# yangzichuang/TextSummarization-On-Flink

Measured on AMD Instinct MI355X. Metric: train_tokens_per_sec, higher is better.
Workload: dtype bf16; 1 GPU; model=pointer-generator+coverage hidden=256 emb=128 enc=400 dec=100 vocab=50000, global_batch=256, per_gpu_batch=256, seq_len=400->100, parallelism=dp1, backend=none, grad_allreduce=none, graph=True, persistent_lstm=True, proj_attn=True, skip_pad_steps=True, decoder_row_groups=2

## Files before the change

### csrc/bindings.cpp

```cpp
#include <torch/library.h>
#include <ATen/ATen.h>
#include <c10/hip/HIPStream.h>
#include <algorithm>
#include <optional>

#include "launchers.h"

using at::Tensor;
using OT = std::optional<Tensor>;

namespace {

hipStream_t stream() { return c10::hip::getCurrentHIPStream().stream(); }

void chk(const Tensor& t, at::ScalarType dt, const char* name) {
  TORCH_CHECK(t.is_cuda(), name, " must be a GPU tensor");
  TORCH_CHECK(t.scalar_type() == dt, name, " has dtype ", t.scalar_type(), ", expected ", dt);
  TORCH_CHECK(t.is_contiguous(), name, " must be contiguous");
}
template <typename T>
T* P(const Tensor& t) { return reinterpret_cast<T*>(t.data_ptr()); }
template <typename T>
T* PO(const OT& t) { return t.has_value() && t->defined() ? reinterpret_cast<T*>(t->data_ptr()) : nullptr; }
void numel_eq(const Tensor& t, int64_t n, const char* name) {
// ... 444 lines not shown
}


void dec_cell_fwd(const Tensor& XG, const OT& ctxp, const Tensor& hprev, const Tensor& cprev, const Tensor& WcT,
                  const Tensor& c_out, const Tensor& cb_out, const Tensor& hb_out, const Tensor& act, int64_t B,
                  int64_t H, int64_t A, const OT& dlen, int64_t step) {
  chk(XG, F32, "XG"); chk(hprev, BF, "hprev"); chk(cprev, F32, "cprev"); chk(WcT, BF, "WcT"); chk(c_out, F32, "c_out");
  chk(cb_out, BF, "cb_out"); chk(hb_out, BF, "hb_out"); chk(act, F32, "act");
  TORCH_CHECK(H % 32 == 0 && A % 32 == 0, "dims must be multiples of 32");
  numel_eq(XG, B * 4 * H, "XG"); chko(ctxp, BF, B * A, "ctxp"); numel_eq(hprev, B * H, "hprev");
  numel_eq(cprev, B * H, "cprev"); numel_eq(WcT, 4 * H * (A + H), "WcT"); numel_eq(c_out, B * H, "c_out");
  numel_eq(cb_out, B * H, "cb_out"); numel_eq(hb_out, B * H, "hb_out"); numel_eq(act, B * 4 * H, "act");
  chko(dlen, I32, B, "dlen");
  launch_dec_cell_fwd(P<float>(XG), PO<bf16>(ctxp), P<bf16>(hprev), P<float>(cprev), P<bf16>(WcT), P<float>(c_out),
                      P<bf16>(cb_out), P<bf16>(hb_out), P<float>(act), B, H, A, PO<int>(dlen), (int)step, stream());
}

void dec_sproj(const Tensor& cb, const Tensor& hb, const Tensor& WsT, const Tensor& bs, const Tensor& s_out, int64_t B,
               int64_t H, int64_t A, const OT& dlen, int64_t step) {
  chk(cb, BF, "cb"); chk(hb, BF, "hb"); chk(WsT, BF, "WsT"); chk(bs, F32, "bs"); chk(s_out, F32, "s_out");
  TORCH_CHECK(H % 32 == 0 && A % 16 == 0, "bad dims");
  numel_eq(cb, B * H, "cb"); numel_eq(hb, B * H, "hb"); numel_eq(WsT, A * 2 * H, "WsT"); numel_eq(bs, A, "bs");
  numel_eq(s_out, B * A, "s_out"); chko(dlen, I32, B, "dlen");
  launch_dec_sproj(P<bf16>(cb), P<bf16>(hb), P<bf16>(WsT), P<float>(bs), P<float>(s_out), B, H, A, PO<int>(dlen),
                   (int)step, stream());
}

void dec_bwd_cell(const Tensor& ds, const Tensor& Ws, const OT& dC_dir, const OT& dH_dir, const Tensor& dh_rec,
                  const Tensor& dc_carry, const Tensor& act, const Tensor& c_now, const Tensor& c_prev,
                  const Tensor& dz, int64_t B, int64_t H, int64_t A, const OT& dlen, int64_t step) {
  chk(ds, F32, "ds"); chk(Ws, BF, "Ws"); chk(dh_rec, F32, "dh_rec"); chk(dc_carry, F32, "dc_carry");
  chk(act, F32, "act"); chk(c_now, F32, "c_now"); chk(c_prev, F32, "c_prev"); chk(dz, BF, "dz");
  TORCH_CHECK(H % 16 == 0 && A % 32 == 0, "bad dims");
  numel_eq(ds, B * A, "ds"); numel_eq(Ws, 2 * H * A, "Ws"); chko(dC_dir, F32, B * H, "dC_dir");
  chko(dH_dir, F32, B * H, "dH_dir"); numel_eq(dh_rec, B * H, "dh_rec"); numel_eq(dc_carry, B * H, "dc_carry");
  numel_eq(act, B * 4 * H, "act"); numel_eq(c_now, B * H, "c_now"); numel_eq(c_prev, B * H, "c_prev");
  numel_eq(dz, B * 4 * H, "dz"); chko(dlen, I32, B, "dlen");
  launch_dec_bwd_cell(P<float>(ds), P<bf16>(Ws), PO<float>(dC_dir), PO<float>(dH_dir), P<float>(dh_rec),
                      P<float>(dc_carry), P<float>(act), P<float>(c_now), P<float>(c_prev), P<bf16>(dz), B, H, A,
                      PO<int>(dlen), (int)step, stream());
}

void dec_bwd_dz(const Tensor& dz, const Tensor& Wbig, const OT& dX_dir, const OT& dCTX_dir_prev, const Tensor& dx_out,
                const OT& dctx_prev_out, const Tensor& dh_rec, int64_t B, int64_t E, int64_t H, int64_t A,
                const OT& dlen, int64_t step) {
  chk(dz, BF, "dz"); chk(Wbig, BF, "Wbig"); chk(dx_out, F32, "dx_out"); chk(dh_rec, F32, "dh_rec");
  TORCH_CHECK(E % 16 == 0 && H % 32 == 0 && A % 16 == 0, "bad dims");
  numel_eq(dz, B * 4 * H, "dz"); numel_eq(Wbig, (E + H + A) * 4 * H, "Wbig");
  chko(dX_dir, F32, B * E, "dX_dir"); chko(dCTX_dir_prev, F32, B * A, "dCTX_dir_prev");
  numel_eq(dx_out, B * E, "dx_out"); chko(dctx_prev_out, F32, B * A, "dctx_prev_out");
  numel_eq(dh_rec, B * H, "dh_rec"); chko(dlen, I32, B, "dlen");
  launch_dec_bwd_dz(P<bf16>(dz), P<bf16>(Wbig), PO<float>(dX_dir), PO<float>(dCTX_dir_prev), P<float>(dx_out),
                    PO<float>(dctx_prev_out), P<float>(dh_rec), B, E, H, A, PO<int>(dlen), (int)step, stream());
}

void ptr_loss(const Tensor& logits, const OT& bias, const Tensor& target, const Tensor& rowg, const OT& pgen,
              const OT& attn, const Tensor& ext, const Tensor& lens, const Tensor& loss_row, const OT& dlogits,
              const OT& dpre, const OT& dA, int64_t N, int64_t B, int64_t T, int64_t V) {
  const bool lbf = logits.scalar_type() == at::kBFloat16;
  chk(logits, lbf ? BF : F32, "logits"); chk(target, I32, "target"); chk(rowg, F32, "rowg"); chk(ext, I32, "ext");
  chk(lens, I32, "lens"); chk(loss_row, F32, "loss_row");
  TORCH_CHECK(lbf != bias.has_value(), "bf16 logits carry their bias (pass None); fp32 logits need the bias");
  chko(bias, F32, V, "bias");
  numel_eq(logits, N * V, "logits"); numel_eq(target, N, "target"); numel_eq(rowg, N, "rowg");
  numel_eq(ext, B * T, "ext"); numel_eq(lens, B, "lens"); numel_eq(loss_row, N, "loss_row");
  TORCH_CHECK(N % B == 0, "N must be D*B");
  chko(pgen, F32, N, "pgen"); chko(attn, F32, N * T, "attn"); chko(dlogits, BF, N * V, "dlogits");
  chko(dpre, F32, N, "dpre"); chko(dA, F32, N * T, "dA");
  TORCH_CHECK(!PO<float>(pgen) || (PO<float>(attn) && (!PO<bf16>(dlogits) || (PO<float>(dpre) && PO<float>(dA)))),
              "pointer mode needs attn, and dpre/dA when computing grads");
  if (lbf) {
    TORCH_CHECK(V <= ptr_loss_bf16_max_vocab(), "bf16 ptr_loss: V <= 65536");
    launch_ptr_loss_bf16(P<bf16>(logits), P<int>(target), P<float>(rowg), PO<float>(pgen), PO<float>(attn),
                         P<int>(ext), P<int>(lens), P<float>(loss_row), PO<bf16>(dlogits), PO<float>(dpre),
                         PO<float>(dA), N, B, T, V, stream());
    return;
  }
  launch_ptr_loss(P<float>(logits), P<float>(*bias), P<int>(target), P<float>(rowg), PO<float>(pgen), PO<float>(attn),
                  P<int>(ext), P<int>(lens), P<float>(loss_row), PO<bf16>(dlogits), PO<float>(dpre), PO<float>(dA), N,
                  B, T, V, stream());
}

int64_t wgrad_tt_ws(int64_t M, int64_t N, int64_t K) {
  if (wgrad_tt_ok((int)M, (int)N, (int)K))
    return wgrad_tt_direct((int)M, (int)N, (int)K, false, false) ? 1
                                                                 : (int64_t)wgrad_tt_splits((int)M, (int)N, (int)K) * M * N;
  if (wgrad_tt_ok((int)N, (int)M, (int)K)) return (int64_t)wgrad_tt_splits((int)N, (int)M, (int)K) * M * N;
  return 0;
}
bool wgrad_tt(const Tensor& a, const Tensor& b, const Tensor& out, const Tensor& ws, bool acc) {
  TORCH_CHECK(a.dim() == 2 && b.dim() == 2 && out.dim() == 2, "wgrad_tt: 2-D views");
  TORCH_CHECK(a.is_cuda() && b.is_cuda() && out.is_cuda() && ws.is_cuda(), "wgrad_tt: GPU tensors");
  TORCH_CHECK(a.scalar_type() == BF && b.scalar_type() == BF && out.scalar_type() == F32 && ws.scalar_type() == F32,
              "wgrad_tt: bf16, bf16 -> fp32");
  TORCH_CHECK(a.stride(1) == 1 && b.stride(1) == 1 && out.stride(1) == 1 && ws.is_contiguous(), "wgrad_tt: unit column stride");
  const int64_t K = a.size(0), M = a.size(1), N = b.size(1), nv = out.size(1);
  TORCH_CHECK(b.size(0) == K && out.size(0) == M && nv <= N, "wgrad_tt: shapes");
  if (!(a.stride(0) % 8 == 0 && b.stride(0) % 8 == 0 && (uintptr_t)a.data_ptr() % 16 == 0 &&
        (uintptr_t)b.data_ptr() % 16 == 0))
    return false;
  const bool plain = wgrad_tt_ok((int)M, (int)N, (int)K), swapped = !plain && wgrad_tt_ok((int)N, (int)M, (int)K);
  if (!plain && !(swapped && nv == N)) return false;
  if (nv != N && (nv % 4 != 0)) return false;
  const bool direct = plain && wgrad_tt_direct((int)M, (int)N, (int)K, false, acc);
  const int64_t need = direct ? 0 : (int64_t)wgrad_tt_splits((int)(plain ? M : N), (int)(plain ? N : M), (int)K) * M * N;
  if (ws.numel() < need) {
// ... 699 lines not shown
  auto part = at::empty({S, Kt}, gw.options());
  auto cpart = at::empty({(int64_t)colsum_det_chunks((int)S, (int)Kt), Kt}, gw.options());
  launch_pgen_bwd(P<float>(ctx), P<float>(c), P<bf16>(h), P<float>(x), P<float>(dpre), P<float>(gw), P<float>(part),
                  P<float>(cpart), N, A, H, E, stream());
}

void pgen_dirs(const Tensor& dpre, const Tensor& w, const Tensor& dctx, const Tensor& dc, const Tensor& dh,
               const Tensor& dx, const OT& gb, int64_t N, int64_t A, int64_t H, int64_t E) {
  chk(dpre, F32, "dpre"); chk(w, F32, "w"); chk(dctx, F32, "dctx"); chk(dc, F32, "dc"); chk(dh, F32, "dh");
  chk(dx, F32, "dx"); chko(gb, F32, 1, "gb");
  numel_eq(dpre, N, "dpre"); numel_eq(w, A + 2 * H + E, "w"); numel_eq(dctx, N * A, "dctx"); numel_eq(dc, N * H, "dc");
  numel_eq(dh, N * H, "dh"); numel_eq(dx, N * E, "dx");
  launch_pgen_dirs(P<float>(dpre), P<float>(w), P<float>(dctx), P<float>(dc), P<float>(dh), P<float>(dx), PO<float>(gb),
                   (int)N, (int)A, (int)H, (int)E, stream());
}

}

TORCH_LIBRARY(tsamd, m) {
  m.def("lstm_enc_fwd_step", &lstm_enc_fwd_step);
  m.def("lstm_enc_bwd_step", &lstm_enc_bwd_step);
  m.def("lstm_persistent_grid", &lstm_persistent_grid_op);
  m.def("lstm_persistent_capacity", &lstm_persistent_capacity_op);
  m.def("lstm_persistent_launches", &lstm_persistent_launches_op);
  m.def("rs_fwd", &rs_fwd);
  m.def("vocab_topk_pg", &vocab_topk_pg);
  m.def("rs_bwd", &rs_bwd);
  m.def("lstm_persistent_xbuf", &lstm_persistent_xbuf_op);
  m.def("lstm_fwd_persistent", &lstm_fwd_persistent);
  m.def("lstm_fwd_persistent_fx", &lstm_fwd_persistent_fx);
  m.def("lstm_persistent_fx_ok", &lstm_persistent_fx_ok_op);
  m.def("lstm_bwd_persistent", &lstm_bwd_persistent);
  m.def("attn_score", &attn_score);
  m.def("attn_softmax_ctx", &attn_softmax_ctx);
  m.def("attn_bwd_step", &attn_bwd_step);
  m.def("attn_row_ok", &attn_row_ok);
  m.def("attn_fwd_row", &attn_fwd_row);
  m.def("attn_bwd_row", &attn_bwd_row);
  m.def("attn_rowp_ok", &attn_rowp_ok);
  m.def("attn_fwd_rowp", &attn_fwd_rowp);
  m.def("dec_persistent_ok", &dec_persistent_ok_op);
  m.def("dec_persistent_grid", &dec_persistent_grid_op);
  m.def("dec_persistent_capacity", &dec_persistent_capacity_op);
  m.def("dec_persistent_xbuf", &dec_persistent_xbuf_op);
  m.def("dec_persistent_stamps", &dec_persistent_stamps_op);
  m.def("dec_fwd_persistent", &dec_fwd_persistent);
  m.def("attn_bwd_rowp", &attn_bwd_rowp);
  m.def("attn_bwd_feat", &attn_bwd_feat);
  m.def("attn_chunks", &attn_chunks);
  m.def("dec_cell_fwd", &dec_cell_fwd);
  m.def("dec_sproj", &dec_sproj);
  m.def("dec_bwd_cell", &dec_bwd_cell);
  m.def("dec_bwd_dz", &dec_bwd_dz);
  m.def("ptr_loss", &ptr_loss);
  m.def("wgrad_tn", &wgrad_tn);
  m.def("wgrad_tt", &wgrad_tt);
  m.def("ctx_bmm_ok", &ctx_bmm_ok_op);
  m.def("ctx_fwd", &ctx_fwd);
  m.def("ctx_da", &ctx_da);
  m.def("ctx_de", &ctx_de);
  m.def("wgrad_tt_ws", &wgrad_tt_ws);
  m.def("pgen_dirs", &pgen_dirs);
  m.def("pack_cast", &pack_cast);
  m.def("pack_max_jobs", &pack_max_jobs_op);
  m.def("pack_job_cols", &pack_job_cols_op);
  m.def("debug_enabled", &debug_enabled);
  m.def("debug_status", &debug_status);
  m.def("debug_clear", &debug_clear);
  m.def("gemm_bt_ok", &gemm_bt_ok);
  m.def("gemm_bt", &gemm_bt);
  m.def("gemm_bt_splitk_ws", &gemm_bt_splitk_ws);
  m.def("gemm_bt_splitk", &gemm_bt_splitk);
  m.def("gemm_bt_merge", &gemm_bt_merge);
  m.def("cu_hold_max_lds", &cu_hold_max_lds_op);
  m.def("cu_hold", &cu_hold);
  m.def("tanh_eval", &tanh_eval);
  m.def("tanh_tput", &tanh_tput);
  m.def("vocab_train_tiles", &vocab_train_tiles_op);
  m.def("vocab_train_fwd", &vocab_train_fwd);
  m.def("vocab_train_bwd", &vocab_train_bwd);
  m.def("emb_grad", &emb_grad);
  m.def("emb_grad_sorted", &emb_grad_sorted);
  m.def("emb_grad_det", &emb_grad_det);
  m.def("emb_grad_det_chunks", &emb_grad_det_chunks_op);
  m.def("to_step_frame", &to_step_frame);
  m.def("from_step_frame", &from_step_frame);
  m.def("transpose_bta", &transpose_bta);
  m.def("tr01", &tr01);
  m.def("linear2_pair", &linear2_pair);
  m.def("cast_colsum", &cast_colsum);
  m.def("colsum", &colsum);
  m.def("step_frame_hop", &step_frame_hop);
  m.def("ptr_rowfin", &ptr_rowfin);
  m.def("clip_adagrad", &clip_adagrad);
  m.def("opt_parts", &opt_parts);
  m.def("final_topk", &final_topk);
  m.def("final_topk_wide", &final_topk_wide);
  m.def("topk_parts", &topk_parts);
  m.def("beam_step", &beam_step);
  m.def("beam_step_wide", &beam_step_wide);
  m.def("beam_step_ng", &beam_step_ng);
  m.def("beam_step_pen", &beam_step_pen);
  m.def("cov_penalty", &cov_penalty);
  m.def("beam_gather", &beam_gather);
  m.def("linear2", &linear2);
  m.def("pgen", &pgen);
// ... 15 lines not shown
```

### csrc/kernels/launchers.h

```cpp
#pragma once
#include <hip/hip_runtime.h>
typedef __bf16 bf16;

void launch_lstm_enc_fwd_step(const float* gx, const float* bias, const bf16* Wt, bf16* hs, float* cs, float* acts, bf16* out,
                              const int* lens, int s, int T, int B, int H, hipStream_t st);
void launch_lstm_enc_bwd_step(bf16* dz, const bf16* Wn, const float* dout, const float* dh_fin, float* dc_carry,
                              const float* acts, const float* cs, const int* lens, int s, int T, int B, int H,
                              hipStream_t st);

void launch_attn_score(const bf16* F, const float* s, const float* v, const float* wc, const float* cov,
                       const int* lens, float* e, int B, int T, int A, int rep, hipStream_t st);
void launch_attn_softmax_ctx(const float* e, const bf16* E, const int* lens, const float* cov, float* a_out,
                             float* cov_out, float* covloss, float* ctx, bf16* ctx_bf, int B, int T, int A, int rep,
                             hipStream_t st);
int attn_nchunk(int T);
void launch_attn_bwd_step(const bf16* E, const bf16* F, const float* s, const float* v, const float* wc,
                          const float* cov, const float* a, const float* dctx, const float* ctx, const float* Ga,
                          const float* dcov_next, const float* gcl, const int* lens, float* de_out, float* ds,
                          float* dcov_out, int B, int T, int A, hipStream_t st);
void launch_attn_bwd_feat(const bf16* F, const float* S_all, const float* v, const float* wc, const float* cov_all,
                          const float* de_all, const int* lens, bf16* dF, float* dv, float* dwc, int D, int B, int T,
                          int A, int nslot, hipStream_t st, const int* dlen = nullptr);

bool attn_row_supported(int A, int T);
void launch_attn_fwd_row_probe(const bf16* F, const bf16* E, const float* s, const float* v, const float* wc,
                               const float* cov, const int* lens, float* a_out, float* ctx, int B, int T, int rep,
                               int probe, hipStream_t st);
void launch_attn_fwd_row(const bf16* F, const bf16* E, const float* s, const float* v, const float* wc,
                         const float* cov, const int* lens, float* a_out, float* cov_out, float* covloss, float* ctx,
                         bf16* ctx_bf, int B, int T, int A, int rep, hipStream_t st, const int* cg = nullptr,
                         const float* asrc = nullptr, float* cov_keep = nullptr);
void launch_attn_bwd_row(const bf16* E, const bf16* F, const float* s, const float* v, const float* wc,
                         const float* cov, const float* a, const float* dctx, const float* ctx, const float* Ga,
                         const float* dcov_next, const float* gcl, const int* lens, float* de_out, float* ds,
                         float* dcov_out, int B, int T, int A, hipStream_t st);

bool attn_rowp_supported(int A, int T, int EG);
void launch_attn_fwd_rowp(const bf16* F, const bf16* G, const float* s, const float* v, const float* wc,
                          const float* cov, const int* lens, float* a_out, float* cov_out, float* covloss, float* gx,
                          bf16* gx_bf, int B, int T, int A, const int* dlen, int step, hipStream_t st,
                          bf16* a_bf = nullptr);
void launch_attn_bwd_rowp(const bf16* G, const bf16* F, const float* s, const float* v, const float* wc,
                          const float* cov, const float* a, const float* dx, const float* gv, const float* Ga,
                          const float* dcov_next, const float* gcl, const int* lens, float* de_out, float* ds,
                          float* dcov_out, int B, int T, int A, const int* dlen, int step, hipStream_t st);

void launch_dec_cell_fwd(const float* XG, const bf16* ctxp, const bf16* hprev, const float* cprev, const bf16* WcT,
                         float* c_out, bf16* cb_out, bf16* hb_out, float* act, int B, int H, int A, const int* dlen,
                         int step, hipStream_t st);
void launch_dec_cell_fwd_beam(const int* gidx, const int* latest, const float* XGtab, const bf16* ctxp,
                              const bf16* hprev, const float* cprev, const bf16* WcT, float* c_out, bf16* cb_out,
                              bf16* hb_out, int* step, int B, int H, int A, int V, int unk, hipStream_t st);
void launch_beam_sproj_xmerge(const bf16* cb, const bf16* hb, const bf16* WsT, const float* bs, float* s_out,
                              const bf16* ctx_src, const bf16* WicT, const float* Xtab, const int* gidx,
                              const int* latest, float* x_out, int B, int H, int A, int E, int V, int unk,
                              hipStream_t st);
void launch_dec_sproj(const bf16* cb, const bf16* hb, const bf16* WsT, const float* bs, float* s_out, int B, int H,
                      int A, const int* dlen, int step, hipStream_t st);
bool dec_persistent_shape_ok(int H, int E, int A, int B, int T);
int dec_persistent_grid(int B);
int dec_persistent_capacity();
size_t dec_persistent_xbuf_elems(int B);
int dec_persistent_stamps_into(unsigned* buf);
void launch_dec_fwd_persistent(const float* XG, const bf16* KcT, const bf16* WsT, const float* bs, float* Cst, bf16* Cb,
                               bf16* Hb, float* ACT, float* S, const bf16* F, const bf16* G, const float* v,
                               const float* wc, float* COV, const int* lens, float* ATT, bf16* ATTb, float* covloss,
                               float* GV, bf16* GVb, const int* dlen, unsigned long long* xbuf, unsigned* err, int B,
                               int T, int D, hipStream_t st);
void launch_dec_bwd_cell(const float* ds, const bf16* Ws, const float* dC_dir, const float* dH_dir,
                         const float* dh_rec, float* dc_carry, const float* act, const float* c_now,
                         const float* c_prev, bf16* dz, int B, int H, int A, const int* dlen, int step,
                         hipStream_t st);
void launch_dec_bwd_dz(const bf16* dz, const bf16* Wbig, const float* dX_dir, const float* dCTX_dir_prev,
                       float* dx_out, float* dctx_prev_out, float* dh_rec, int B, int E, int H, int A,
                       const int* dlen, int step, hipStream_t st);

void launch_ptr_loss_bf16(const bf16* logits, const int* target, const float* rowg, const float* pgen,
                          const float* attn, const int* ext, const int* lens, float* loss_row, bf16* dlogits,
                          float* dpre, float* dA, int N, int B, int T, int V, hipStream_t st);
int ptr_loss_bf16_max_vocab();
void launch_ptr_loss(const float* logits, const float* bias, const int* target, const float* rowg, const float* pgen, const float* attn,
                     const int* ext, const int* lens, float* loss_row, bf16* dlogits, float* dpre, float* dA, int N,
                     int B, int T, int V, hipStream_t st);

void launch_clip_adagrad(float* w, float* acc, const float* g, long n, float* part, float lr, float max_norm,
                         float gscale, float* norm_out, int* flag, const int* skip, hipStream_t st);
int opt_nparts();

void launch_final_topk(const float* logits, const float* bias, const float* pgen, const float* attn, const int* ext,
                       const int* lens, int* out_ids, float* out_lp, float* part_ms, float* part_v, int* part_i, int R,
                       int V, int T, int K, int beam, hipStream_t st, bool wide = false);
#define NG_BAN_MAX 4096
struct NgSeq {
  int* seq[2];
  int P;
  int n;
};
struct BeamPen {
  const float* inv_len;
  const float* cpen;
  float beta;
  float* key_sum;
  float* res_lp;
};
void launch_cov_penalty(const float* cov, const float* att, const int* lens, float* cpen, int R, int T, int beam,
                        hipStream_t st, const float* a0 = nullptr);
int topk_split(int V);
void launch_beam_step(const int* top_ids, const float* top_lp, float* lp_sum, int* latest, int* gidx, int* tok_hist,
                      int* par_hist, int* done, int* res_count, float* res_score, int* res_len, int* res_step,
                      int* res_par, int* step, unsigned* ctr, const float* att, float* att_hist, const float* pg,
                      float* pg_hist, int T, int Na, int beam, int K, int stop_id, int min_dec, int max_dec,
                      hipStream_t st, const NgSeq* ng = nullptr, const BeamPen* pen = nullptr);
void launch_beam_step_wide(const int* top_ids, const float* top_lp, float* lp_sum, int* latest, int* gidx,
                           int* tok_hist, int* par_hist, int* done, int* res_count, float* res_score, int* res_len,
                           int* res_step, int* res_par, const int* step, const float* att, float* att_hist,
                           const float* pg, float* pg_hist, int T, int Na, int beam, int K, int stop_id, int min_dec,
                           int max_dec, hipStream_t st, const NgSeq* ng = nullptr, const BeamPen* pen = nullptr);
void launch_beam_gather(const int* gidx, const int* latest, const float* c_src, const bf16* h_src,
                        const float* ctx_src, const float* a_src, const float* cov_src, const float* XGtab,
                        const float* Xtab, float* c_out, bf16* h_out, float* ctx_out, bf16* ctxb_out, float* cov_out,
                        float* XG_out, float* x_out, int R, int H, int A, int T, int E, int V, int unk,
                        int* step, hipStream_t st);
void launch_linear2(const bf16* a1, int K1, const bf16* a2, int K2, const bf16* Wt, const float* bias,
                    const float* add, float* out, bf16* outb, int B, int N, hipStream_t st);
void launch_linear2_pair(const bf16* a1, int K1, const bf16* a2, int K2, const bf16* Wt, const float* bias,
                         const float* add, float* out, bf16* outb, int N, const bf16* c1, int L1, const bf16* c2,
                         int L2, const bf16* Vt, const float* vbias, const float* vadd, float* vout, bf16* voutb,
                         int M, int B, hipStream_t st);
// ... 119 lines not shown
```

### textsummarization_on_flink_amd/models/engine_config.py

```python
from __future__ import annotations

import os
from dataclasses import dataclass, fields, replace
from typing import Mapping, Optional


def _flag(env: Mapping[str, str], name: str, default: bool) -> bool:
    v = env.get(name, "")
    return default if v == "" else v != "0"


def _tri(env: Mapping[str, str], name: str) -> Optional[bool]:
    v = env.get(name, "")
    return None if v == "" else v != "0"


@dataclass(frozen=True)
class EngineConfig:
    persistent_lstm: bool = True
    dec_persistent: bool = True
    row_attn: Optional[bool] = None
    split: int = 0
    split_bwd: int = 0
    fused_vocab_train: bool = True
    fused_vocab_decode: bool = True
    proj_attn: bool = True
    skip_pad_steps: bool = True
    decode_row_attn: bool = True
    compact_vocab_grad: bool = True
    defer_wgrad: bool = True
    deterministic: bool = False

    @classmethod
    def from_env(cls, env: Optional[Mapping[str, str]] = None, **overrides) -> "EngineConfig":
        env = os.environ if env is None else env
        cfg = cls(
            persistent_lstm=_flag(env, "TSAMD_LSTM_PERSISTENT", True),
            dec_persistent=_flag(env, "TSAMD_DEC_PERSISTENT", True),
            row_attn=_tri(env, "TSAMD_ROW_ATTN"),
            split=int(env.get("TSAMD_SPLIT", "0") or 0),
            split_bwd=int(env.get("TSAMD_SPLIT_BWD", "0") or 0),
            fused_vocab_train=_flag(env, "TSAMD_FUSED_VOCAB_TRAIN", True),
            fused_vocab_decode=_flag(env, "TSAMD_FUSED_VOCAB", True),
            proj_attn=_flag(env, "TSAMD_PROJ_ATTN", True),
            skip_pad_steps=_flag(env, "TSAMD_SKIP_PAD_STEPS", True),
            decode_row_attn=_flag(env, "TSAMD_DEC_ROW_ATTN", True),
            compact_vocab_grad=_flag(env, "TSAMD_COMPACT_VOCAB_GRAD", True),
            defer_wgrad=_flag(env, "TSAMD_DEFER_WGRAD", True),
            deterministic=_flag(env, "TSAMD_DETERMINISTIC", False),
        )
        return replace(cfg, **overrides) if overrides else cfg

    def as_dict(self):
        return {f.name: getattr(self, f.name) for f in fields(self)}


DEC_PERSISTENT_TEAM = 16


def dec_persistent_grid(B: int) -> int:
    if B < 16 or B % 16:
        return 0
    return 8 * DEC_PERSISTENT_TEAM * (-(-(B // 16) // 8))


def dec_persistent_eligible(H: int, E: int, A: int, B: int, T: int, proj_attn: bool, row_attn: bool,
                            world: int = 1, capacity: int = 0, reserve_cus: int = 0) -> bool:
    if not (proj_attn and row_attn):
        return False
    if (H, E, A) != (256, 128, 512) or B < 16 or B % 16 or not 1 <= T <= 2048:
        return False
    grid = dec_persistent_grid(B)
    cap = capacity - (reserve_cus if world > 1 else 0)
    return 0 < grid <= cap
```

### textsummarization_on_flink_amd/models/pointer_generator.py

```python
from __future__ import annotations


import os
from typing import Dict, List, Optional

import numpy as np
import torch

from ..ops import ops as _ops
from ..parallel.rccl_env import rccl_cu_reserve
from .engine_config import EngineConfig, dec_persistent_eligible
from .params import DEC, P, FlatParams, enc_prefix

BF = torch.bfloat16
F32 = torch.float32

EMB = f"{P}/embedding/embedding"
RC, RH = f"{P}/reduce_final_st/w_reduce_c", f"{P}/reduce_final_st/w_reduce_h"
BRC, BRH = f"{P}/reduce_final_st/bias_reduce_c", f"{P}/reduce_final_st/bias_reduce_h"
WH, VATT, WCOV = f"{DEC}/W_h", f"{DEC}/v", f"{DEC}/coverage/w_c"
LIN_M, LIN_B = f"{DEC}/Linear/Matrix", f"{DEC}/Linear/Bias"
CELL_K, CELL_B = f"{DEC}/lstm_cell/kernel", f"{DEC}/lstm_cell/bias"
ATT_M, ATT_B = f"{DEC}/Attention/Linear/Matrix", f"{DEC}/Attention/Linear/Bias"
PG_M, PG_B = f"{DEC}/calculate_pgen/Linear/Matrix", f"{DEC}/calculate_pgen/Linear/Bias"
OUT_M, OUT_B = f"{DEC}/AttnOutputProjection/Linear/Matrix", f"{DEC}/AttnOutputProjection/Linear/Bias"
OW, OV = f"{P}/output_projection/w", f"{P}/output_projection/v"


class LstmHandoffError(RuntimeError):
    """A persistent-LSTM launch timed out in a hand-off (a workgroup was not co-resident)."""


def enc_k(layer, d):
    return f"{enc_prefix(layer)}/bidirectional_rnn/{d}/lstm_cell/kernel"


def enc_b(layer, d):
    return f"{enc_prefix(layer)}/bidirectional_rnn/{d}/lstm_cell/bias"


BLT = os.environ.get("TSAMD_BLT", "1") != "0"
BLT_WGRAD = BLT and os.environ.get("TSAMD_BLT_WGRAD", "0") == "1"
BLT_VDW = BLT and os.environ.get("TSAMD_BLT_VOCAB_DW", "0") == "1"
VOCAB_PAD = os.environ.get("TSAMD_VOCAB_PAD", "1") != "0"
CTX_NATIVE = os.environ.get("TSAMD_CTX_NATIVE", "1") != "0"
DE_BF16 = os.environ.get("TSAMD_DE_BF16", "1") != "0"
VOCAB_DW_SPLIT_MIN = 1e12
VOCAB_DW_SIDE = os.environ.get("TSAMD_VOCAB_DW_SIDE", "0") == "1"


GEMM_BT = os.environ.get("TSAMD_GEMM_BT", "table")
_BT_PICK: Dict[tuple, bool] = {}
_BT_TIMES: Dict[tuple, tuple] = {}
DX_MERGE = os.environ.get("TSAMD_DX_MERGE", "1") != "0"
LSTM_FX = os.environ.get("TSAMD_LSTM_FX", "1") != "0"
K2LOG2E = 2.8853900817779268
FRAME_SLACK = 1.25


def _aligned(t: torch.Tensor) -> bool:
    return t.stride(-1) == 1 and (t.dim() < 2 or t.stride(0) % 8 == 0) and t.data_ptr() % 16 == 0


def _bt_ok(out, sa, ta, Bt, beta, bias) -> bool:
# ... 370 lines not shown
        self.fused_vocab = cfg.fused_vocab_train and H in (128, 256, 512)
        if self.fused_vocab:
            N = D * B
            w["vpart"] = z(int(self.k.vocab_train_tiles(V, H)) * N * 2)
            for n in ("zg", "lse", "pv", "alpha"):
                w[n] = z(N)
            w["dbias"] = z(V)
            w["vstate"] = z((N + 31) // 32, dt=torch.int32)
        self.Vp = -(-V // 128) * 128 if (self.fused_vocab and VOCAB_PAD) else V
        self.ctx_native = CTX_NATIVE and self.dev.type == "cuda" and bool(self.k.ctx_bmm_ok(B, T, D, A))
        w["logits"] = z(D * B, self.Vp, dt=BF)
        if self.Vp != V and self.det:
            w["dbias_p"] = z(self.Vp)
        w["dlogits"] = w["logits"]
        self.vocab_buckets = sorted({max(1, -(-nblk * f // 8)) for f in (4, 5, 6, 7, 8)})
        self.nbk = self.vocab_buckets[-1]
        w["dpre"] = z(D, B)
        w["dA"] = z(D, B, T)
        w["DCTX"] = z(D, B, A)
        w["DX"] = z(D, B, E)
        w["DZ"] = z(D, B, 4 * H, dt=BF)
        w["DS"] = z(D, B, A)
        w["d_emb_dec"] = z(D * B, E)
        w["out_f32"] = z(D * B, H)
        if self.hps.pointer_gen:
            w["dC_dir"] = z(D, B, H)
            w["dX_dir"] = z(D, B, E)
        w["DE"] = z(D, B, T)
        w["dcov"] = z(2, B, T)
        w["dh_rec"] = z(B, H)
        w["dc_carry"] = z(B, H)
        w["dF"] = z(B, T, A, dt=BF)
        w["ATTb"] = z(D, B, T, dt=BF)
        w["DCTXb"] = z(D, B, A, dt=BF)
        self.de_bf16 = DE_BF16 and self.ctx_native and self.persistent_lstm
        self._dE = z(B, T, A, dt=BF if self.de_bf16 else F32)
        self.split_vocab_dw = False
        self._pending_dw = None
        nfeat = ((T + 15) // 16) * B
        nslot = 1 << (nfeat - 1).bit_length() if self.det else 32
        w["dv"] = z(nslot, A)
        w["dwc"] = z(nslot, A)
        if self.det:
            nc = int(self.k.emb_grad_det_chunks(B * T + D * B))
            w["emb_pf"] = z(nc, E)
            w["emb_pl"] = z(nc, E)
        w["opt_part"] = z(int(self.k.opt_parts()))
        w["gnorm"] = z(1)
        w["nan_flag"] = z(1, dt=torch.int32)
        self.w = w

    def _dec_persistent_select(self) -> None:
        k = self.k
        cap = int(k.dec_persistent_capacity()) if (self.cfg.dec_persistent and self.proj_attn) else 0
        self.dec_persistent = self.cfg.dec_persistent and dec_persistent_eligible(
            self.H, self.E, self.A, self.B, self.T, self.proj_attn, self.row_attn, self.world, cap,
            rccl_cu_reserve())
        if self.dec_persistent and getattr(self, "_dec_xbuf", None) is None:
            self._dec_xbuf = torch.zeros(int(k.dec_persistent_xbuf(self.B)), dtype=torch.long, device=self.dev)

    def set_world(self, world: int) -> None:
        self.world = int(world)
        self._dec_persistent_select()

    def check_lstm_err(self) -> None:
        code = int(self.w["lstm_err"].item())
        if code == 3:
            raise LstmHandoffError("persistent decoder forward hand-off timed out (code 3: a workgroup was not "
                                   "co-resident); results of that launch were discarded -- set "
                                   "TSAMD_DEC_PERSISTENT=0 (EngineConfig.dec_persistent)")
        if code:
            raise LstmHandoffError(f"persistent LSTM hand-off timed out (code {code}: a workgroup was not "
                                   "co-resident); results of that launch were discarded -- set "
                                   "TSAMD_LSTM_PERSISTENT=0 (EngineConfig.persistent_lstm)")

    def pack(self):
        jobs = getattr(self, "_pack_jobs", None)
        if jobs is not None:
            E = self.E
            torch.mm(self.p[LIN_M][E:], self.p[CELL_K][:E], out=self._wcomb)
            self.k.pack_cast(jobs, self._pack_total)
            return
        self._pack_torch()
        if self.p.flat.is_cuda:
            self._build_pack_jobs()

    def _pack_job_pairs(self):
        p, E, H, A, pk, f32 = self.p, self.E, self.H, self.A, self.pk, self.f32
        M, K, W = p[LIN_M], p[CELL_K], self._wcomb
        pairs = [(pk["emb"], p[EMB])]
        for layer in range(self.L):
            din = E if layer == 0 else A
            for di, d in enumerate(("fw", "bw")):
                Kd = p[enc_k(layer, d)]
                pairs += [(pk[f"enc{layer}_Kx{di}"], Kd[:din]),
                          (pk[f"enc{layer}_Kxi{di}"].view(din, H, 4), Kd[:din].view(din, 4, H).permute(0, 2, 1)),
                          (pk[f"enc{layer}_KxiT{di}"].view(H, 4, din), Kd[:din].view(din, 4, H).permute(2, 1, 0)),
                          (pk[f"enc{layer}_Wn"][di], Kd[din:]), (pk[f"enc{layer}_Wt"][di], Kd[din:].t()),
                          (f32[f"enc{layer}_b"][di], p[enc_b(layer, d)])]
                if layer > 0:
                    pairs.append((pk[f"enc{layer}_Kx01"][:, di * 4 * H:(di + 1) * 4 * H], Kd[:din]))
        pairs += [(pk["Wh"], p[WH].reshape(A, A)),
                  (pk["WhK"], p[WH].reshape(A, A), K2LOG2E), (pk["WhKT"], p[WH].reshape(A, A).t(), K2LOG2E),
                  (pk["lin_embT"], M[:E].t()),
                  (pk["RC"], p[RC]), (pk["RH"], p[RH]), (pk["RCt"], p[RC].t()),
                  (pk["RHt"], p[RH].t()), (pk["lin_emb"], M[:E]), (pk["Wic"], M[E:]), (pk["WicT"], M[E:].t()),
                  (pk["cell_x"], K[:E]), (pk["KcT"], K.t()), (pk["WcT2"][:, :A], W.t()), (pk["WcT2"][:, A:], K[E:].t()),
                  (pk["Wbig"][:E + H], K), (pk["Wbig"][E + H:], W), (pk["Ws"], p[ATT_M]), (pk["WsT"], p[ATT_M].t()),
                  (pk["OUTm"], p[OUT_M]), (pk["OUTmT"], p[OUT_M].t()), (pk["ow"], p[OW]), (pk["ovb"], p[OV])]
        if "owT" in pk:
            pairs.append((pk["owT"], p[OW].t()))
        return pairs

    def _build_pack_jobs(self):
        E = self.E
        self._wcomb = torch.mm(self.p[LIN_M][E:], self.p[CELL_K][:E])
        rows, blk = [], 0
        for dst, src, *scale in self._pack_job_pairs():
            assert dst.shape == src.shape and src.dtype == F32 and dst.dtype in (BF, F32) and dst.dim() <= 3, \
# ... 529 lines not shown
        if not self.row_attn_bwd:
            w["DS"].zero_()
        Ga = w["dA"] if hps.pointer_gen else None
        def chain(r0, r1):
            Bg, rs = r1 - r0, slice(r0, r1)
            for t in reversed(range(D)):
                dcov_next = dcov[(t + 1) % 2][rs] if (cov and t < D - 1) else None
                cov_t = w["COV"][t][rs] if (cov and t > 0) else None
                gcl_t = w["gcl"][t][rs] if cov else None
                ga_t = Ga[t][rs] if Ga is not None else None
                if self.row_attn_bwd:
                    k.attn_bwd_row(enc_out[rs], F[rs], w["S"][t][rs], v, wc, cov_t, w["ATT"][t][rs], w["DCTX"][t][rs],
                                   w["CTX"][t][rs], ga_t, dcov_next, gcl_t, lens[rs], w["DE"][t][rs], w["DS"][t][rs],
                                   dcov[t % 2][rs] if cov else None, Bg, T, A)
                else:
                    k.attn_bwd_step(enc_out[rs], F[rs], w["S"][t][rs], v, wc, cov_t, w["ATT"][t][rs], w["DCTX"][t][rs],
                                    w["CTX"][t][rs], ga_t, dcov_next, gcl_t, lens[rs], w["DE"][t][rs], w["DS"][t][rs],
                                    dcov[t % 2][rs] if cov else None, Bg, T, A)
                k.dec_bwd_cell(w["DS"][t][rs], self.pk["Ws"], dC_dir[t][rs] if dC_dir is not None else None,
                               dH_dir[t][rs], w["dh_rec"][rs], w["dc_carry"][rs], w["ACT"][t][rs], w["Cst"][t + 1][rs],
                               w["Cst"][t][rs], w["DZ"][t][rs], Bg, H, A, None, 0)
                k.dec_bwd_dz(w["DZ"][t][rs], self.pk["Wbig"], dX_dir[t][rs] if dX_dir is not None else None,
                             dCTX_dir[t - 1][rs] if t > 0 else None, w["DX"][t][rs],
                             w["DCTX"][t - 1][rs] if t > 0 else None, w["dh_rec"][rs], Bg, E, H, A, None, 0)

        self._row_groups(chain, self.split_bwd)
        self._backward_mid_rest(Hn, wg, run)

    def _backward_mid_proj(self, dCTX_dir, dH_dir, dC_dir, dX_dir, Hn, wg, run):
        k, w, hps = self.k, self.w, self.hps
        B, T, D, E, H, A = self.B, self.T, self.D, self.E, self.H, self.A
        N = D * B
        cov = hps.coverage
        enc_out, lens, F, G = self.enc[-1]["out"], w["enc_lens"], w["F"], w["Genc"]
        v, wc = self.f32["v"], self.f32["wc"]
        w["DCTXb"].copy_(dCTX_dir)
        Ga = w["dA"]
        if self.ctx_native:
            k.ctx_da(w["DCTXb"], enc_out, Ga, B, T, D, A, bool(hps.pointer_gen))
        else:
            da = w["bd_tmp"][:B * D * T].view(B, D, T)
            torch.bmm(w["DCTXb"].permute(1, 0, 2), enc_out.transpose(1, 2), out_dtype=F32, out=da)
            if T % 4 == 0:
                k.tr01(da, Ga, None, B, D, T, bool(hps.pointer_gen))
            elif hps.pointer_gen:
                Ga.add_(da.transpose(0, 1))
            else:
                Ga.copy_(da.transpose(0, 1))
        w["dh_rec"].zero_()
        w["dc_carry"].zero_()
        dcov = w["dcov"]
        Kc = self.pk["Wbig"][:E + H]
        dlen = w["dlen"] if self.skip_pad else None

        def chain(r0, r1):
            Bg, rs = r1 - r0, slice(r0, r1)
            dl = dlen[rs] if dlen is not None else None
            for t in reversed(range(D)):
                nxt = t < D - 1
                k.attn_bwd_rowp(G[rs], F[rs], w["S"][t][rs], v, wc, w["COV"][t][rs] if (cov and t > 0) else None,
                                w["ATT"][t][rs], w["DX"][t + 1][rs] if nxt else None, w["GV"][t][rs],
                                Ga[t][rs], dcov[(t + 1) % 2][rs] if (cov and nxt) else None,
                                w["gcl"][t][rs] if cov else None, lens[rs], w["DE"][t][rs], w["DS"][t][rs],
                                dcov[t % 2][rs] if cov else None, Bg, T, A, dl, t)
                k.dec_bwd_cell(w["DS"][t][rs], self.pk["Ws"], dC_dir[t][rs] if dC_dir is not None else None,
                               dH_dir[t][rs], w["dh_rec"][rs], w["dc_carry"][rs], w["ACT"][t][rs], w["Cst"][t + 1][rs],
                               w["Cst"][t][rs], w["DZ"][t][rs], Bg, H, A, dl, t)
                k.dec_bwd_dz(w["DZ"][t][rs], Kc, dX_dir[t][rs] if dX_dir is not None else None, None,
                             w["DX"][t][rs], None, w["dh_rec"][rs], Bg, E, H, 0, dl, t)

        self._row_groups(chain, self.split_bwd)
        if dCTX_dir is not w["DCTX"]:
            w["DCTX"].copy_(dCTX_dir)
        if D > 1:
            dctx = w["DCTX"][:D - 1].view((D - 1) * B, A)
            dxb = w["DXb"][1:].view((D - 1) * B, E)
            dxb.copy_(w["DX"][1:].view((D - 1) * B, E))
            gemm(dctx, dxb, self.pk["WicT"], 1.0, bt=self.pk["Wic"])
        self._backward_mid_rest(Hn, wg, run)

    def _backward_mid_rest(self, Hn, wg, run):
        k, w, hps, p = self.k, self.w, self.hps, self.p
        B, T, D, E, H, A = self.B, self.T, self.D, self.E, self.H, self.A
        N = D * B
        g = p.g
        cov = hps.coverage
        v, wc = self.f32["v"], self.f32["wc"]
        lens, F = w["enc_lens"], w["F"]
        emb_dec = self._emb_dec

        DXb = self._cast_colsum(w["DX"].view(N, E), g(LIN_B))
        gemm(w["d_emb_dec"], DXb, self.pk["lin_emb"].t())

        def dec_wgrad():
            DZ = w["DZ"].view(N, 4 * H)
            gk = g(CELL_K)
            wg(gk[:E], w["Xb"].view(N, E), DZ)
            wg(gk[E:], w["Hb"][:D].reshape(N, H), DZ)
            k.colsum(DZ, g(CELL_B), N, 4 * H, False)
            gl = g(LIN_M)
            wg(gl[:E], emb_dec, DXb)
            gl[E:].zero_()
            if D > 1:
                wg(gl[E:], w["CTXb"][:D - 1].reshape((D - 1) * B, A), DXb[B:])
            DSb = self._cast_colsum(w["DS"].view(N, A), g(ATT_B))
            gs = g(ATT_M)
            wg(gs[:H], w["Cb"][1:].reshape(N, H), DSb)
            wg(gs[H:], Hn, DSb)
        run(dec_wgrad)
        w["dv"].zero_()
        w["dwc"].zero_()
        k.attn_bwd_feat(F, w["S"], v, wc, w["COV"][:D] if cov else None, w["DE"], lens, w["dF"], w["dv"],
                        w["dwc"] if cov else None, D, B, T, A, w["dlen"] if self.skip_pad else None)
        k.colsum(w["dv"], g(VATT).view(A), w["dv"].shape[0], A, False)
        if cov:
            k.colsum(w["dwc"], g(WCOV).view(A), w["dwc"].shape[0], A, False)
        dFb = w["dF"].view(B * T, A)
# ... 116 lines not shown
```

Before: 8.088 million tokens/s.

## Fuse decoder backward cell and dz projection into one co-resident kernel

Adds a fused HIP kernel that computes the decoder LSTM backward cell (ds·Ws projection, gate gradients, carry) and then the dz·Kc projection for dx/dh_rec in a single launch per reverse step. Teams of workgroups exchange dz granules through a tagged global buffer with spin-wait hand-off instead of relying on a second kernel launch. This removes one launch and a global round-trip per decoder step. In exchange it requires all workgroups to be co-resident, adds a timeout error path (code 4), and is restricted to H=256, E=128, A=512.

```diff
diff --git a/csrc/bindings.cpp b/csrc/bindings.cpp
--- a/csrc/bindings.cpp
+++ b/csrc/bindings.cpp
@@ -520,6 +520,36 @@
   numel_eq(dh_rec, B * H, "dh_rec"); chko(dlen, I32, B, "dlen");
   launch_dec_bwd_dz(P<bf16>(dz), P<bf16>(Wbig), PO<float>(dX_dir), PO<float>(dCTX_dir_prev), P<float>(dx_out),
                     PO<float>(dctx_prev_out), P<float>(dh_rec), B, E, H, A, PO<int>(dlen), (int)step, stream());
+}
+
+bool dec_bwd_fused_ok_op(int64_t H, int64_t E, int64_t A, int64_t B) {
+  return dec_bwd_fused_shape_ok((int)H, (int)E, (int)A, (int)B);
+}
+int64_t dec_bwd_fused_grid_op(int64_t B) { return dec_bwd_fused_grid((int)B); }
+int64_t dec_bwd_fused_xbuf_op(int64_t B) { return (int64_t)dec_bwd_fused_xbuf_elems((int)B); }
+void dec_bwd_celldz(const Tensor& ds, const Tensor& Ws, const OT& dC_dir, const OT& dH_dir, const Tensor& dh_rec,
+                    const Tensor& dc_carry, const Tensor& act, const Tensor& c_now, const Tensor& c_prev,
+                    const Tensor& dz, const Tensor& Kc, const OT& dX_dir, const Tensor& dx_out, const OT& dlen,
+                    const Tensor& xbuf, const Tensor& err, int64_t B, int64_t E, int64_t H, int64_t A, int64_t step,
+                    int64_t tag) {
+  TORCH_CHECK(dec_bwd_fused_shape_ok((int)H, (int)E, (int)A, (int)B), "dec_bwd_celldz: unsupported shape");
+  TORCH_CHECK(tag >= 1 && tag <= 0x7fffffff, "dec_bwd_celldz: tag = D - step must be positive");
+  TORCH_CHECK(dec_bwd_fused_grid((int)B) <= dec_persistent_capacity(),
+              "dec_bwd_celldz: the grid would not be co-resident on this device");
+  chk(ds, F32, "ds"); chk(Ws, BF, "Ws"); chk(dh_rec, F32, "dh_rec"); chk(dc_carry, F32, "dc_carry");
+  chk(act, F32, "act"); chk(c_now, F32, "c_now"); chk(c_prev, F32, "c_prev"); chk(dz, BF, "dz");
+  chk(Kc, BF, "Kc"); chk(dx_out, F32, "dx_out"); chk(xbuf, at::kLong, "xbuf"); chk(err, I32, "err");
+  numel_eq(ds, B * A, "ds"); numel_eq(Ws, 2 * H * A, "Ws"); chko(dC_dir, F32, B * H, "dC_dir");
+  chko(dH_dir, F32, B * H, "dH_dir"); numel_eq(dh_rec, B * H, "dh_rec"); numel_eq(dc_carry, B * H, "dc_carry");
+  numel_eq(act, B * 4 * H, "act"); numel_eq(c_now, B * H, "c_now"); numel_eq(c_prev, B * H, "c_prev");
+  numel_eq(dz, B * 4 * H, "dz"); numel_eq(Kc, (E + H) * 4 * H, "Kc"); chko(dX_dir, F32, B * E, "dX_dir");
+  numel_eq(dx_out, B * E, "dx_out"); chko(dlen, I32, B, "dlen");
+  numel_eq(xbuf, (int64_t)dec_bwd_fused_xbuf_elems((int)B), "xbuf");
+  launch_dec_bwd_celldz(P<float>(ds), P<bf16>(Ws), PO<float>(dC_dir), PO<float>(dH_dir), P<float>(dh_rec),
+                        P<float>(dc_carry), P<float>(act), P<float>(c_now), P<float>(c_prev), P<bf16>(dz),
+                        P<bf16>(Kc), PO<float>(dX_dir), P<float>(dx_out), PO<int>(dlen),
+                        (unsigned long long*)xbuf.data_ptr(), (unsigned*)err.data_ptr(), (int)B, (int)step,
+                        (unsigned)tag, stream());
 }
 
 void ptr_loss(const Tensor& logits, const OT& bias, const Tensor& target, const Tensor& rowg, const OT& pgen,
@@ -1325,6 +1355,10 @@
   m.def("dec_sproj", &dec_sproj);
   m.def("dec_bwd_cell", &dec_bwd_cell);
   m.def("dec_bwd_dz", &dec_bwd_dz);
+  m.def("dec_bwd_fused_ok", &dec_bwd_fused_ok_op);
+  m.def("dec_bwd_fused_grid", &dec_bwd_fused_grid_op);
+  m.def("dec_bwd_fused_xbuf", &dec_bwd_fused_xbuf_op);
+  m.def("dec_bwd_celldz", &dec_bwd_celldz);
   m.def("ptr_loss", &ptr_loss);
   m.def("wgrad_tn", &wgrad_tn);
   m.def("wgrad_tt", &wgrad_tt);
diff --git a/csrc/kernels/decoder_bwd_step.hip b/csrc/kernels/decoder_bwd_step.hip
--- /dev/null
+++ b/csrc/kernels/decoder_bwd_step.hip
@@ -0,0 +1,166 @@
+#include "common.h"
+#include "handoff.h"
+#include "launchers.h"
+
+using namespace handoff;
+
+namespace {
+
+constexpr int kH = 256, kE = 128, kA = 512, kNC = 16;
+constexpr int kG = 4 * kH;
+constexpr int kN = kE + kH;
+constexpr int kCols = kN / kNC;
+constexpr int kDzS = kG + 8;
+constexpr int kTeamGranules = 16 * (kG / 2);
+constexpr unsigned kErrCode = 4u;
+constexpr int kSleep = 8;
+static_assert(kN % kNC == 0 && kCols > 16 && kCols <= 32, "two overlapping 16-column tiles per workgroup");
+static_assert(kTeamGranules == 4 * 32 * 64, "sweep: 4 waves x 32 granules per lane");
+
+}
+
+struct DecBwdStepArgs {
+  const float* ds;
+  const bf16* Ws;
+  const float* dC_dir;
+  const float* dH_dir;
+  float* dh_rec;
+  float* dc_carry;
+  const float* act;
+  const float* c_now;
+  const float* c_prev;
+  bf16* dz;
+  const bf16* Kc;
+  const float* dX_dir;
+  float* dx_out;
+  const int* dlen;
+  gu64* xbuf;
+  gu32* err;
+  int B, step;
+  unsigned tag;
+};
+
+__global__ __launch_bounds__(256) void dec_bwd_celldz_kernel(DecBwdStepArgs p) {
+  __shared__ __attribute__((aligned(16))) bf16 dzl[16 * kDzS];
+  __shared__ float red[4 * 2 * 256];
+  int team, j;
+  if (!team_of(kNC, p.B / 16, team, j)) return;
+  const int wid = threadIdx.x >> 6, lane = threadIdx.x & 63;
+  const int l15 = lane & 15, kof = 8 * (lane >> 4);
+  const int r0 = team * 16;
+  const int rl = (lane >> 4) * 4 + wid, r = r0 + rl;
+  const int u = 16 * j + l15;
+  const int na = kCols * j + l15, nb = na + kCols - 16;
+  const bool use_b = l15 >= 32 - kCols;
+  bf16* dzr = p.dz + (size_t)r * kG;
+  auto put = [&](int n, float val, bool live) {
+    if (n < kE) p.dx_out[(size_t)r * kE + n] = val + ((live && p.dX_dir) ? p.dX_dir[(size_t)r * kE + n] : 0.f);
+    else p.dh_rec[(size_t)r * kH + n - kE] = val;
+  };
+  {
+    const int* dlen = p.dlen;
+    if (dlen && __all(p.step >= dlen[r0 + l15])) {
+      dzr[u] = f2bf(0.f); dzr[kH + u] = f2bf(0.f); dzr[2 * kH + u] = f2bf(0.f); dzr[3 * kH + u] = f2bf(0.f);
+      put(na, 0.f, false);
+      if (use_b) put(nb, 0.f, false);
+      return;
+    }
+  }
+  bf16x8 wa[8], wb[8];
+  {
+    const bf16* browa = p.Kc + (size_t)na * kG + kof + wid * (kG / 4);
+    const bf16* browb = p.Kc + (size_t)nb * kG + kof + wid * (kG / 4);
+#pragma unroll
+    for (int i = 0; i < 8; ++i) {
+      wa[i] = ld8(browa + 32 * i);
+      wb[i] = ld8(browb + 32 * i);
+    }
+  }
+  const size_t ri = (size_t)r * kH + u;
+  float dh0, dc0, a4[4], cn, cpv;
+  {
+    dh0 = p.dh_rec[ri] + (p.dH_dir ? p.dH_dir[ri] : 0.f);
+    dc0 = p.dc_carry[ri] + (p.dC_dir ? p.dC_dir[ri] : 0.f);
+    const float* ap = p.act + (size_t)r * kG;
+#pragma unroll
+    for (int g = 0; g < 4; ++g) a4[g] = ap[g * kH + u];
+    cn = p.c_now[ri];
+    cpv = p.c_prev[ri];
+  }
+  float o[2];
+  {
+    const float* arow = p.ds + (size_t)(r0 + l15) * kA + kof;
+    const bf16* bc = p.Ws + (size_t)u * kA + kof;
+    const bf16* bh = p.Ws + (size_t)(kH + u) * kA + kof;
+    const int nst = kA / 32;
+    const int k0 = (wid * nst / 4) * 32, k1 = ((wid + 1) * nst / 4) * 32;
+    f32x4 acc[2] = {f32x4{0, 0, 0, 0}, f32x4{0, 0, 0, 0}};
+    kslice_mma<2>([&](int k) { return ld8f(arow + k); },
+                  [&](int jj, int k) { return ld8((jj == 0 ? bc : bh) + k); }, k0, k1, acc);
+    ksplit_reduce<2>(acc, red, o);
+  }
+  const float dh = dh0 + o[1];
+  float dc = dc0 + o[0];
+  const float ig = a4[0], jg = a4[1], fg = a4[2], og = a4[3];
+  const float tc = ftanh(cn);
+  dc += dh * og * (1.0f - tc * tc);
+  const float dzo = dh * tc * og * (1.0f - og);
+  const float dzi = dc * jg * ig * (1.0f - ig);
+  const float dzj = dc * ig * (1.0f - jg * jg);
+  const float dzf = dc * cpv * fg * (1.0f - fg);
+  const float carry = dc * fg;
+  gu64* tb = p.xbuf + (size_t)team * kTeamGranules;
+  {
+    const bool odd = l15 & 1;
+    const float n0 = dpp_f<DPP_XOR1>(odd ? dzi : dzf), n1 = dpp_f<DPP_XOR1>(odd ? dzj : dzo);
+    gu64* g = tb + rl * (kG / 2) + (odd ? kH : 0) + (u >> 1);
+    store_granule(g, p.tag, odd ? pack_bf2(n0, dzf) : pack_bf2(dzi, n0));
+    store_granule(g + kH / 2, p.tag, odd ? pack_bf2(n1, dzo) : pack_bf2(dzj, n1));
+  }
+  {
+    unsigned v[32];
+#pragma unroll
+    for (int q = 0; q < 32; ++q) v[q] = 0u;
+    bool dead = false;
+    sweep<32, kSleep>(tb, wid * 4 * (kG / 2), p.tag, v, dead, p.err, kErrCode, lane);
+#pragma unroll
+    for (int q = 0; q < 32; ++q)
+      *reinterpret_cast<unsigned*>(dzl + (4 * wid + (q >> 3)) * kDzS + 2 * ((q & 7) * 64 + lane)) = v[q];
+  }
+  p.dc_carry[ri] = carry;
+  dzr[u] = f2bf(dzi); dzr[kH + u] = f2bf(dzj); dzr[2 * kH + u] = f2bf(dzf); dzr[3 * kH + u] = f2bf(dzo);
+  __syncthreads();
+  float o2[2];
+  {
+    const bf16* arow = dzl + l15 * kDzS + kof + wid * (kG / 4);
+    f32x4 acc[2] = {f32x4{0, 0, 0, 0}, f32x4{0, 0, 0, 0}};
+#pragma unroll
+    for (int i = 0; i < 8; ++i) {
+      const bf16x8 a = ld8(arow + 32 * i);
+      acc[0] = mfma16(a, wa[i], acc[0]);
+      acc[1] = mfma16(a, wb[i], acc[1]);
+    }
+    ksplit_reduce<2>(acc, red, o2);
+  }
+  put(na, o2[0], true);
+  if (use_b) put(nb, o2[1], true);
+}
+
+bool dec_bwd_fused_shape_ok(int H, int E, int A, int B) {
+  return H == kH && E == kE && A == kA && B >= 16 && B % 16 == 0;
+}
+
+int dec_bwd_fused_grid(int B) { return B >= 16 && B % 16 == 0 ? 8 * kNC * ((B / 16 + 7) / 8) : 0; }
+
+size_t dec_bwd_fused_xbuf_elems(int B) { return (size_t)(B / 16) * kTeamGranules; }
+
+void launch_dec_bwd_celldz(const float* ds, const bf16* Ws, const float* dC_dir, const float* dH_dir, float* dh_rec,
+                           float* dc_carry, const float* act, const float* c_now, const float* c_prev, bf16* dz,
+                           const bf16* Kc, const float* dX_dir, float* dx_out, const int* dlen,
+                           unsigned long long* xbuf, unsigned* err, int B, int step, unsigned tag, hipStream_t st) {
+  const int grid = dec_bwd_fused_grid(B);
+  if (grid <= 0) return;
+  DecBwdStepArgs p{ds, Ws, dC_dir, dH_dir, dh_rec, dc_carry, act, c_now, c_prev, dz, Kc, dX_dir, dx_out, dlen,
+                   (gu64*)xbuf, (gu32*)err, B, step, tag};
+  hipLaunchKernelGGL(dec_bwd_celldz_kernel, dim3(grid), dim3(256), 0, st, p);
+}
diff --git a/csrc/kernels/launchers.h b/csrc/kernels/launchers.h
--- a/csrc/kernels/launchers.h
+++ b/csrc/kernels/launchers.h
@@ -74,6 +74,13 @@
 void launch_dec_bwd_dz(const bf16* dz, const bf16* Wbig, const float* dX_dir, const float* dCTX_dir_prev,
                        float* dx_out, float* dctx_prev_out, float* dh_rec, int B, int E, int H, int A,
                        const int* dlen, int step, hipStream_t st);
+bool dec_bwd_fused_shape_ok(int H, int E, int A, int B);
+int dec_bwd_fused_grid(int B);
+size_t dec_bwd_fused_xbuf_elems(int B);
+void launch_dec_bwd_celldz(const float* ds, const bf16* Ws, const float* dC_dir, const float* dH_dir, float* dh_rec,
+                           float* dc_carry, const float* act, const float* c_now, const float* c_prev, bf16* dz,
+                           const bf16* Kc, const float* dX_dir, float* dx_out, const int* dlen,
+                           unsigned long long* xbuf, unsigned* err, int B, int step, unsigned tag, hipStream_t st);
 
 void launch_ptr_loss_bf16(const bf16* logits, const int* target, const float* rowg, const float* pgen,
                           const float* attn, const int* ext, const int* lens, float* loss_row, bf16* dlogits,
diff --git a/textsummarization_on_flink_amd/models/engine_config.py b/textsummarization_on_flink_amd/models/engine_config.py
--- a/textsummarization_on_flink_amd/models/engine_config.py
+++ b/textsummarization_on_flink_amd/models/engine_config.py
@@ -19,6 +19,7 @@
 class EngineConfig:
     persistent_lstm: bool = True
     dec_persistent: bool = True
+    dec_bwd_fused: bool = True
     row_attn: Optional[bool] = None
     split: int = 0
     split_bwd: int = 0
@@ -37,6 +38,7 @@
         cfg = cls(
             persistent_lstm=_flag(env, "TSAMD_LSTM_PERSISTENT", True),
             dec_persistent=_flag(env, "TSAMD_DEC_PERSISTENT", True),
+            dec_bwd_fused=_flag(env, "TSAMD_DEC_BWD_FUSED", True),
             row_attn=_tri(env, "TSAMD_ROW_ATTN"),
             split=int(env.get("TSAMD_SPLIT", "0") or 0),
             split_bwd=int(env.get("TSAMD_SPLIT_BWD", "0") or 0),
@@ -73,3 +75,13 @@
     grid = dec_persistent_grid(B)
     cap = capacity - (reserve_cus if world > 1 else 0)
     return 0 < grid <= cap
+
+
+def dec_bwd_fused_eligible(H: int, E: int, A: int, B: int, proj_attn: bool, groups: int = 1, world: int = 1,
+                           capacity: int = 0, reserve_cus: int = 0) -> bool:
+    if not proj_attn or (H, E, A) != (256, 128, 512):
+        return False
+    if groups < 1 or B < 16 * groups or B % (16 * groups):
+        return False
+    cap = capacity - (reserve_cus if world > 1 else 0)
+    return 0 < groups * dec_persistent_grid(B // groups) <= cap
diff --git a/textsummarization_on_flink_amd/models/pointer_generator.py b/textsummarization_on_flink_amd/models/pointer_generator.py
--- a/textsummarization_on_flink_amd/models/pointer_generator.py
+++ b/textsummarization_on_flink_amd/models/pointer_generator.py
@@ -9,7 +9,7 @@
 
 from ..ops import ops as _ops
 from ..parallel.rccl_env import rccl_cu_reserve
-from .engine_config import EngineConfig, dec_persistent_eligible
+from .engine_config import EngineConfig, dec_bwd_fused_eligible, dec_persistent_eligible
 from .params import DEC, P, FlatParams, enc_prefix
 
 BF = torch.bfloat16
@@ -486,12 +486,17 @@
 
     def _dec_persistent_select(self) -> None:
         k = self.k
-        cap = int(k.dec_persistent_capacity()) if (self.cfg.dec_persistent and self.proj_attn) else 0
+        want = (self.cfg.dec_persistent or self.cfg.dec_bwd_fused) and self.proj_attn
+        cap = int(k.dec_persistent_capacity()) if want else 0
         self.dec_persistent = self.cfg.dec_persistent and dec_persistent_eligible(
             self.H, self.E, self.A, self.B, self.T, self.proj_attn, self.row_attn, self.world, cap,
             rccl_cu_reserve())
         if self.dec_persistent and getattr(self, "_dec_xbuf", None) is None:
             self._dec_xbuf = torch.zeros(int(k.dec_persistent_xbuf(self.B)), dtype=torch.long, device=self.dev)
+        self.dec_bwd_fused = self.cfg.dec_bwd_fused and dec_bwd_fused_eligible(
+            self.H, self.E, self.A, self.B, self.proj_attn, self.split_bwd, self.world, cap, rccl_cu_reserve())
+        if self.dec_bwd_fused and getattr(self, "_dec_bwd_xbuf", None) is None:
+            self._dec_bwd_xbuf = torch.zeros(int(k.dec_bwd_fused_xbuf(self.B)), dtype=torch.long, device=self.dev)
 
     def set_world(self, world: int) -> None:
         self.world = int(world)
@@ -499,6 +504,10 @@
 
     def check_lstm_err(self) -> None:
         code = int(self.w["lstm_err"].item())
+        if code == 4:
+            raise LstmHandoffError("fused decoder reverse step hand-off timed out (code 4: a workgroup was not "
+                                   "co-resident); results of that launch were discarded -- set "
+                                   "TSAMD_DEC_BWD_FUSED=0 (EngineConfig.dec_bwd_fused)")
         if code == 3:
             raise LstmHandoffError("persistent decoder forward hand-off timed out (code 3: a workgroup was not "
                                    "co-resident); results of that launch were discarded -- set "
@@ -1134,10 +1143,15 @@
         dcov = w["dcov"]
         Kc = self.pk["Wbig"][:E + H]
         dlen = w["dlen"] if self.skip_pad else None
+        fused = self.dec_bwd_fused
+        if fused:
+            self._dec_bwd_xbuf.zero_()
+            gpt = self._dec_bwd_xbuf.numel() // (B // 16)
 
         def chain(r0, r1):
             Bg, rs = r1 - r0, slice(r0, r1)
             dl = dlen[rs] if dlen is not None else None
+            xb = self._dec_bwd_xbuf[r0 // 16 * gpt:r1 // 16 * gpt] if fused else None
             for t in reversed(range(D)):
                 nxt = t < D - 1
                 k.attn_bwd_rowp(G[rs], F[rs], w["S"][t][rs], v, wc, w["COV"][t][rs] if (cov and t > 0) else None,
@@ -1145,6 +1159,13 @@
                                 Ga[t][rs], dcov[(t + 1) % 2][rs] if (cov and nxt) else None,
                                 w["gcl"][t][rs] if cov else None, lens[rs], w["DE"][t][rs], w["DS"][t][rs],
                                 dcov[t % 2][rs] if cov else None, Bg, T, A, dl, t)
+                if fused:
+                    k.dec_bwd_celldz(w["DS"][t][rs], self.pk["Ws"], dC_dir[t][rs] if dC_dir is not None else None,
+                                     dH_dir[t][rs], w["dh_rec"][rs], w["dc_carry"][rs], w["ACT"][t][rs],
+                                     w["Cst"][t + 1][rs], w["Cst"][t][rs], w["DZ"][t][rs], Kc,
+                                     dX_dir[t][rs] if dX_dir is not None else None, w["DX"][t][rs], dl, xb,
+                                     w["lstm_err"], Bg, E, H, A, t, D - t)
+                    continue
                 k.dec_bwd_cell(w["DS"][t][rs], self.pk["Ws"], dC_dir[t][rs] if dC_dir is not None else None,
                                dH_dir[t][rs], w["dh_rec"][rs], w["dc_carry"][rs], w["ACT"][t][rs], w["Cst"][t + 1][rs],
                                w["Cst"][t][rs], w["DZ"][t][rs], Bg, H, A, dl, t)
```

Result: no change. 8.118 million tokens/s, median of 6 (+0.4%).
